# waldstein94/Stratified-Transformer

Measured on AMD Instinct MI355X. Metric: points/sec through StratifiedAttention fwd+bwd, 100k-pt scene, higher is better.
Workload: dtype f32

## Files before the change

stratified_transformer_amd/csrc/cell_attn.hip:

```cpp
#include "cell_common.h"

namespace p2 {


template <typename T>
__device__ __forceinline__ void stage_table_t(T *lds, const T *__restrict__ tab, int L, int h, int head) {
    const int total = 3 * L * 16;
    for (int x = threadIdx.x; x < total; x += blockDim.x) {
        const int i = x % 16, r = (x / 16) % L, ax = x / (16 * L);
        lds[x] = tab[(((size_t)r * h + head) * 16 + i) * 3 + ax];
    }
}
template <int TS, typename T>
__device__ __forceinline__ void stage_tables(T *lds, const T *__restrict__ table_q, const T *__restrict__ table_k, const T *__restrict__ table_v, int L,
                                             int h, int head) {
    stage_table_t<T>(lds, table_q, L, h, head);
    stage_table_t<T>(lds + TS, table_k, L, h, head);
    stage_table_t<T>(lds + 2 * TS, table_v, L, h, head);
    __syncthreads();
}

template <int LCAP>
struct TabGeo {
    static constexpr int TS = 3 * LCAP * 16;
    static constexpr size_t bytes(size_t elem) { return (size_t)3 * TS * elem; }
};
struct RowOff {
    int o0, o1, o2;
};
__device__ __forceinline__ RowOff row_off(unsigned w, int L, int c) {
    RowOff r;
    r.o0 = (int)(w & 255u) * 16 + 4 * c;
    r.o1 = (int)(L + ((w >> 8) & 255u)) * 16 + 4 * c;
    r.o2 = (int)(2 * L + ((w >> 16) & 255u)) * 16 + 4 * c;
    return r;
}
template <int OFF>
__device__ __forceinline__ float4 tsum_at(const float *lds, RowOff r) {
    return add4(add4(*reinterpret_cast<const float4 *>(lds + OFF + r.o0), *reinterpret_cast<const float4 *>(lds + OFF + r.o1)),
                *reinterpret_cast<const float4 *>(lds + OFF + r.o2));
}

struct Rows3 {
    float4 a, b, c;
};
template <int OFF, typename T>
__device__ __forceinline__ Rows3 rows_at(const T *lds, RowOff r) {
    Rows3 x;
    x.a = ld_row4(lds + OFF + r.o0);
    x.b = ld_row4(lds + OFF + r.o1);
    x.c = ld_row4(lds + OFF + r.o2);
    return x;
}
typedef float f32x2c __attribute__((ext_vector_type(2)));
__device__ __forceinline__ float4 padd4(float4 a, float4 b) {
    const f32x2c lo = f32x2c{a.x, a.y} + f32x2c{b.x, b.y}, hi = f32x2c{a.z, a.w} + f32x2c{b.z, b.w};
    return make_float4(lo.x, lo.y, hi.x, hi.y);
}
__device__ __forceinline__ float4 pfma4(float s, float4 a, float4 acc) {
    const f32x2c ss = f32x2c{s, s};
    const f32x2c lo = __builtin_elementwise_fma(ss, f32x2c{a.x, a.y}, f32x2c{acc.x, acc.y});
    const f32x2c hi = __builtin_elementwise_fma(ss, f32x2c{a.z, a.w}, f32x2c{acc.z, acc.w});
    return make_float4(lo.x, lo.y, hi.x, hi.y);
}
__device__ __forceinline__ float4 rsum(Rows3 r) { return padd4(padd4(r.a, r.b), r.c); }
__device__ __forceinline__ f32x2c pdot_acc(float4 a, float4 b, f32x2c acc) {
    acc = __builtin_elementwise_fma(f32x2c{a.x, a.y}, f32x2c{b.x, b.y}, acc);
    return __builtin_elementwise_fma(f32x2c{a.z, a.w}, f32x2c{b.z, b.w}, acc);
}
__device__ __forceinline__ float pdot4(float4 a, float4 b) {
    const f32x2c r = pdot_acc(a, b, f32x2c{0.f, 0.f});
    return r.x + r.y;
}

template <int NPMAX, typename F>
__device__ __forceinline__ void dispatch_passes(int np, F f) {
    if (np <= 2) f(std::integral_constant<int, 2>{});
    else if (np == 3) f(std::integral_constant<int, 3>{});
    else if (np == 4 || NPMAX <= 4) f(std::integral_constant<int, 4>{});
    else if constexpr (NPMAX > 4) {
        if (np <= 6) f(std::integral_constant<int, 6>{});
        else f(std::integral_constant<int, 8>{});
    }
}

template <typename TT, bool PK>
struct LaneCtx {
    const TT *lds;
    int L, lane, p, c, head, h, C, hoff, rs_packed;
    float qscale;
    __device__ __forceinline__ int rs() const { return PK ? rs_packed : C; }
    template <typename RT>
    __device__ __forceinline__ float4 q_row4(const RT *q, int i) const {
        if constexpr (PK) return scaled_row4<RT>(q + (size_t)i * rs_packed + hoff, qscale);
        else return ld_row4(q + (size_t)i * C + hoff);
    }
};
template <typename TT, bool PK>
__device__ __forceinline__ LaneCtx<TT, PK> make_lane_ctx(const TT *lds, int h, int L, int rs, float qscale) {
    LaneCtx<TT, PK> x;
    x.lds = lds;
    x.L = L;
    x.h = h;
    x.head = blockIdx.y;
    x.C = h * 16;
    x.rs_packed = rs;
    x.qscale = qscale;
    x.lane = threadIdx.x & 63;
    x.p = x.lane >> 2;
    x.c = x.lane & 3;
    x.hoff = x.head * 16 + 4 * x.c;
    return x;
}

template <int NPA, typename RT, typename T, bool PK>
__device__ __forceinline__ void load_key_rows(const LaneCtx<T, PK> &x, const CellBufs &cb, const RT *__restrict__ rows, int j0, int nvalid,
                                              float4 (&r4)[NPA]) {
    unsigned keys[NPA];
    bload_words<NPA>(cb.key, (j0 + x.p * NPA) * 4, keys);
#pragma unroll
    for (int t = 0; t < NPA; t++) {
        const float4 r = ld_row4(rows + (size_t)keys[t] * x.rs() + x.hoff);
        r4[t] = t < nvalid ? r : make_float4(0.f, 0.f, 0.f, 0.f);
    }
}

template <int NPA, int TS, typename RT, typename T, bool PK>
__device__ __forceinline__ void fwd_sweep_logits(const LaneCtx<T, PK> &x, const CellTask &ct, const CellBufs &cb, rsrc_t rs_p,
                                                 const RT *__restrict__ q, const RT *__restrict__ k, float *__restrict__ ml,
                                                 int ch, bool single, int j0, int nkc) {
    const int p = x.p, c = x.c;
    const int nvalid = min(max(nkc - p * NPA, 0), NPA);
    float4 k4[NPA];
    load_key_rows<NPA, RT, T, PK>(x, cb, k, j0, nvalid, k4);
    int ids = (int)bload_u32(cb.qid, x.lane * 4);
    int i_nx = __builtin_amdgcn_readlane(ids, 0);
    float4 q4_nx = x.q_row4(q, i_nx);
    unsigned w_nx[NPA];
    bload_words<NPA>(cb.rel, (j0 + p * NPA) * 4, w_nx);
    for (int il = 0; il < ct.nq; il++) {
        const int i = i_nx;
        const float4 q4 = q4_nx;
        unsigned w[NPA];
#pragma unroll
        for (int t = 0; t < NPA; t++) w[t] = w_nx[t];
        const int roff = (il * ct.nk + j0 + p * NPA) * 4;
        if (((il + 1) & 63) == 0) ids = (int)bload_u32(cb.qid, (il + 1 + x.lane) * 4);
        i_nx = __builtin_amdgcn_readlane(ids, (il + 1) & 63);
        q4_nx = x.q_row4(q, i_nx);
        bload_words<NPA>(cb.rel, roff + ct.nk * 4, w_nx);
        float lg[NPA];
        float mx = -INFINITY;
        RowOff ro = row_off(w[0], x.L, c);
        Rows3 rq = rows_at<0, T>(x.lds, ro), rk = rows_at<TS, T>(x.lds, ro);
#pragma unroll
        for (int t = 0; t < NPA; t++) {
            Rows3 rq1 = rq, rk1 = rk;
            if (t + 1 < NPA) {
                ro = row_off(w[t + 1], x.L, c);
                rq1 = rows_at<0, T>(x.lds, ro);
                rk1 = rows_at<TS, T>(x.lds, ro);
            }
            const f32x2c d2 = pdot_acc(k4[t], rsum(rk), pdot_acc(q4, rsum(rq), pdot_acc(q4, k4[t], f32x2c{0.f, 0.f})));
            const float s = quad_sum(d2.x + d2.y);
            lg[t] = (t < nvalid && !(w[t] >> 31)) ? s : -INFINITY;
            mx = fmaxf(mx, lg[t]);
            rq = rq1;
            rk = rk1;
            __builtin_amdgcn_sched_barrier(0);
        }
        mx = slots_max16(mx);
        if (single) {
            float sum = 0.f;
#pragma unroll
            for (int t = 0; t < NPA; t++) {
                lg[t] = __expf(lg[t] - mx);
                sum += lg[t];
            }
            const float inv = 1.0f / slots_sum16(sum);
#pragma unroll
            for (int t = 0; t < NPA; t++) lg[t] *= inv;
            if (c == 0) bstore_floats<NPA>(rs_p, roff, lg, nvalid);
        } else {
            float *st = ml + ((size_t)i * x.h + x.head) * 2;
            const float m_old = ch ? st[0] : -INFINITY, l_old = ch ? st[1] : 0.f;
            const float m_new = fmaxf(m_old, mx);
            float sum = 0.f;
#pragma unroll
            for (int t = 0; t < NPA; t++) sum += __expf(lg[t] - m_new);
            if (c == 0) bstore_floats<NPA>(rs_p, roff, lg, nvalid);
            sum = slots_sum16(sum);
            if (x.lane == 0) {
                st[0] = m_new;
                st[1] = (m_old == -INFINITY ? 0.f : l_old * __expf(m_old - m_new)) + sum;
            }
        }
    }
}

template <int NPA, int TS, typename RT, typename T, bool PK>
__device__ __forceinline__ void fwd_sweep_values(const LaneCtx<T, PK> &x, const CellTask &ct, const CellBufs &cb, rsrc_t rs_p,
                                                 const RT *__restrict__ v, const float *__restrict__ ml, float *__restrict__ out,
                                                 int ch, bool single, int j0, int nkc) {
    const int p = x.p, c = x.c;
    const int nvalid = min(max(nkc - p * NPA, 0), NPA);
    float4 v4[NPA];
    load_key_rows<NPA, RT, T, PK>(x, cb, v, j0, nvalid, v4);
    unsigned w_nx[NPA];
    float a_nx[NPA];
    bload_words<NPA>(cb.rel, (j0 + p * NPA) * 4, w_nx);
    bload_floats<NPA>(rs_p, (j0 + p * NPA) * 4, a_nx);
    int ids = (int)bload_u32(cb.qid, x.lane * 4);
    for (int il = 0; il < ct.nq; il++) {
        if (il && (il & 63) == 0) ids = (int)bload_u32(cb.qid, (il + x.lane) * 4);
        const int i = __builtin_amdgcn_readlane(ids, il & 63);
        const int roff = (il * ct.nk + j0 + p * NPA) * 4;
        unsigned w[NPA];
        float a[NPA];
#pragma unroll
        for (int t = 0; t < NPA; t++) {
            w[t] = w_nx[t];
            a[t] = a_nx[t];
        }
        bload_words<NPA>(cb.rel, roff + ct.nk * 4, w_nx);
        bload_floats<NPA>(rs_p, roff + ct.nk * 4, a_nx);
        if (!single) {
            const float *st = ml + ((size_t)i * x.h + x.head) * 2;
            const float m = st[0], inv = 1.0f / st[1];
#pragma unroll
            for (int t = 0; t < NPA; t++) a[t] = __expf(a[t] - m) * inv;
            if (c == 0) bstore_floats<NPA>(rs_p, roff, a, nvalid);
        }
        float4 acc = make_float4(0.f, 0.f, 0.f, 0.f);
        Rows3 rv = rows_at<2 * TS, T>(x.lds, row_off(w[0], x.L, c));
#pragma unroll
        for (int t = 0; t < NPA; t++) {
            Rows3 rv1 = rv;
            if (t + 1 < NPA) rv1 = rows_at<2 * TS, T>(x.lds, row_off(w[t + 1], x.L, c));
            const float at = t < nvalid ? a[t] : 0.f;
            acc = pfma4(at, padd4(rsum(rv), v4[t]), acc);
            rv = rv1;
            __builtin_amdgcn_sched_barrier(0);
        }
        const float4 tot = slots_sum16_4(acc);
        if (p == 0) {
            float *o = out + (size_t)i * x.C + x.hoff;
            stg4(o, ch ? add4(tot, ldg4(o)) : tot);
        }
    }
}

template <int NP, int LCAP, typename RT, typename T, bool PK>
__global__ __launch_bounds__(CA_WAVES * 64) void cell_fwd_kernel(pointops2_cell_plan pl, int h, int L, const RT *__restrict__ q,
                                                                 const RT *__restrict__ k, const RT *__restrict__ v, int rs, float qscale,
                                                                 const T *__restrict__ table_q, const T *__restrict__ table_k,
                                                                 const T *__restrict__ table_v, float *__restrict__ out,
                                                                 float *__restrict__ ml, float *__restrict__ pbuf, size_t plane) {
    constexpr int TS = TabGeo<LCAP>::TS;
    extern __shared__ float lds_raw[];
    T *lds = reinterpret_cast<T *>(lds_raw);
    const LaneCtx<T, PK> x = make_lane_ctx<T, PK>(lds, h, L, rs, qscale);
    const int wave = __builtin_amdgcn_readfirstlane(threadIdx.x >> 6);
    stage_tables<TS, T>(lds, table_q, table_k, table_v, L, h, x.head);
    const int nC = share_count(pl, pl.counts[0]);
    float *pb = pbuf + (size_t)x.head * plane;
    const int slots = gridDim.x * CA_WAVES, slot = blockIdx.x * CA_WAVES + wave;
    for (int round = 0; round * slots < nC; round++) {
        const int task = snake_task(round, slot, slots);
        if (task >= nC) continue;
        const CellTask ct = cell_task(pl, share_task(pl, task));
        const int nch = (ct.nk + 16 * NP - 1) / (16 * NP);
        const CellBufs cb = make_cell_bufs(pl, ct);
        const rsrc_t rs_p = tile_rsrc(pb, ct);
        for (int ch = 0; ch < nch; ch++) {
            const int j0 = ch * 16 * NP, nkc = min(16 * NP, ct.nk - j0);
            dispatch_passes<NP>((nkc + 15) >> 4, [&](auto tag) {
                fwd_sweep_logits<decltype(tag)::value, TS, RT, T, PK>(x, ct, cb, rs_p, q, k, ml, ch, nch == 1, j0, nkc);
            });
        }
        for (int ch = 0; ch < nch; ch++) {
            const int j0 = ch * 16 * NP, nkc = min(16 * NP, ct.nk - j0);
            dispatch_passes<NP>((nkc + 15) >> 4, [&](auto tag) {
                fwd_sweep_values<decltype(tag)::value, TS, RT, T, PK>(x, ct, cb, rs_p, v, ml, out, ch, nch == 1, j0, nkc);
            });
        }
    }
}

template <int NPA, typename T, bool PK>
__device__ __forceinline__ void flush_key_pass(float *scr, float4 acc, rsrc_t rs_key, int j0, int t, int nkc, float *__restrict__ grad,
                                               const LaneCtx<T, PK> &x) {
    *reinterpret_cast<float4 *>(scr + x.p * 16 + 4 * x.c) = acc;
    __builtin_amdgcn_s_waitcnt(0xC07F);
    __builtin_amdgcn_wave_barrier();
#pragma unroll
    for (int kk = 0; kk < 4; kk++) {
        const int s = (x.lane >> 4) + 4 * kk;
        const int jl = s * NPA + t;
        const int key = (int)bload_u32(rs_key, (j0 + jl) * 4);
        if (jl < nkc) unsafeAtomicAdd(grad + (size_t)key * x.rs() + x.head * 16 + (x.lane & 15), scr[s * 16 + (x.lane & 15)]);
    }
    __builtin_amdgcn_s_waitcnt(0xC07F);
    __builtin_amdgcn_wave_barrier();
}

template <int NPA, int TS, typename RT, typename T, bool PK>
__device__ __forceinline__ void bwd_sweep_values(const LaneCtx<T, PK> &x, const CellTask &ct, const CellBufs &cb, rsrc_t rs_p, rsrc_t rs_g,
                                                 float *scr, const float *__restrict__ go, const float *__restrict__ out,
                                                 const RT *__restrict__ v, float *__restrict__ grad_v, int j0, int nkc) {
    const int p = x.p, c = x.c;
    const int nvalid = min(max(nkc - p * NPA, 0), NPA);
    float4 v4[NPA], dv4[NPA];
    load_key_rows<NPA, RT, T, PK>(x, cb, v, j0, nvalid, v4);
#pragma unroll
    for (int t = 0; t < NPA; t++) dv4[t] = make_float4(0.f, 0.f, 0.f, 0.f);
    unsigned w_nx[NPA];
    float a_nx[NPA];
    bload_words<NPA>(cb.rel, (j0 + p * NPA) * 4, w_nx);
    bload_floats<NPA>(rs_p, (j0 + p * NPA) * 4, a_nx);
    int ids = (int)bload_u32(cb.qid, x.lane * 4);
    int i_nx = __builtin_amdgcn_readlane(ids, 0);
    float4 go_nx = ldg4(go + (size_t)i_nx * x.C + x.hoff), o_nx = ldg4(out + (size_t)i_nx * x.C + x.hoff);
    for (int il = 0; il < ct.nq; il++) {
        const int roff = (il * ct.nk + j0 + p * NPA) * 4;
        const float4 go4 = go_nx, o4 = o_nx;
        unsigned w[NPA];
        float a[NPA];
#pragma unroll
        for (int t = 0; t < NPA; t++) {
            w[t] = w_nx[t];
            a[t] = t < nvalid ? a_nx[t] : 0.f;
        }
        if (((il + 1) & 63) == 0) ids = (int)bload_u32(cb.qid, (il + 1 + x.lane) * 4);
        i_nx = __builtin_amdgcn_readlane(ids, (il + 1) & 63);
        go_nx = ldg4(go + (size_t)i_nx * x.C + x.hoff);
        o_nx = ldg4(out + (size_t)i_nx * x.C + x.hoff);
        bload_words<NPA>(cb.rel, roff + ct.nk * 4, w_nx);
        bload_floats<NPA>(rs_p, roff + ct.nk * 4, a_nx);
        const float delta = quad_sum(pdot4(go4, o4));
        float gs[NPA];
        Rows3 rv = rows_at<2 * TS, T>(x.lds, row_off(w[0], x.L, c));
#pragma unroll
        for (int t = 0; t < NPA; t++) {
            Rows3 rv1 = rv;
            if (t + 1 < NPA) rv1 = rows_at<2 * TS, T>(x.lds, row_off(w[t + 1], x.L, c));
            const float ga = quad_sum(pdot4(go4, padd4(rsum(rv), v4[t])));
            gs[t] = a[t] * (ga - delta);
            dv4[t] = pfma4(a[t], go4, dv4[t]);
            rv = rv1;
            __builtin_amdgcn_sched_barrier(0);
        }
        if (c == 0) bstore_floats<NPA>(rs_g, roff, gs, nvalid);
    }
#pragma unroll
    for (int t = 0; t < NPA; t++) flush_key_pass<NPA, T, PK>(scr, dv4[t], cb.key, j0, t, nkc, grad_v, x);
}

template <int NPA, int TS, typename RT, typename T, bool PK>
__device__ __forceinline__ void bwd_sweep_keys(const LaneCtx<T, PK> &x, const CellTask &ct, const CellBufs &cb, rsrc_t rs_g, float *scr,
                                               const RT *__restrict__ q, const RT *__restrict__ k, float *__restrict__ grad_q,
                                               float *__restrict__ grad_k, int ch, int j0, int nkc) {
    const int p = x.p, c = x.c;
    const int nvalid = min(max(nkc - p * NPA, 0), NPA);
    float4 k4[NPA], dk4[NPA];
    load_key_rows<NPA, RT, T, PK>(x, cb, k, j0, nvalid, k4);
#pragma unroll
    for (int t = 0; t < NPA; t++) dk4[t] = make_float4(0.f, 0.f, 0.f, 0.f);
    unsigned w_nx[NPA];
    float g_nx[NPA];
    bload_words<NPA>(cb.rel, (j0 + p * NPA) * 4, w_nx);
    bload_floats<NPA>(rs_g, (j0 + p * NPA) * 4, g_nx);
    int ids = (int)bload_u32(cb.qid, x.lane * 4);
    int i_nx = __builtin_amdgcn_readlane(ids, 0);
    float4 q_nx = x.q_row4(q, i_nx);
    for (int il = 0; il < ct.nq; il++) {
        const int i = i_nx;
        const int roff = (il * ct.nk + j0 + p * NPA) * 4;
        const float4 q4 = q_nx;
        unsigned w[NPA];
        float g[NPA];
#pragma unroll
        for (int t = 0; t < NPA; t++) {
            w[t] = w_nx[t];
            g[t] = t < nvalid ? g_nx[t] : 0.f;
        }
        if (((il + 1) & 63) == 0) ids = (int)bload_u32(cb.qid, (il + 1 + x.lane) * 4);
        i_nx = __builtin_amdgcn_readlane(ids, (il + 1) & 63);
        q_nx = x.q_row4(q, i_nx);
        bload_words<NPA>(cb.rel, roff + ct.nk * 4, w_nx);
        bload_floats<NPA>(rs_g, roff + ct.nk * 4, g_nx);
        float4 dq = make_float4(0.f, 0.f, 0.f, 0.f);
        RowOff ro = row_off(w[0], x.L, c);
        Rows3 rq = rows_at<0, T>(x.lds, ro), rk = rows_at<TS, T>(x.lds, ro);
#pragma unroll
        for (int t = 0; t < NPA; t++) {
            Rows3 rq1 = rq, rk1 = rk;
            if (t + 1 < NPA) {
                ro = row_off(w[t + 1], x.L, c);
                rq1 = rows_at<0, T>(x.lds, ro);
                rk1 = rows_at<TS, T>(x.lds, ro);
            }
            dq = pfma4(g[t], padd4(rsum(rq), k4[t]), dq);
            dk4[t] = pfma4(g[t], padd4(rsum(rk), q4), dk4[t]);
            rq = rq1;
            rk = rk1;
            __builtin_amdgcn_sched_barrier(0);
        }
        float4 tot = slots_sum16_4(dq);
        if constexpr (PK) tot = make_float4(tot.x * x.qscale, tot.y * x.qscale, tot.z * x.qscale, tot.w * x.qscale);
        if (p == 0) {
            float *o = grad_q + (size_t)i * x.rs() + x.hoff;
            stg4(o, ch ? add4(tot, ldg4(o)) : tot);
        }
    }
#pragma unroll
    for (int t = 0; t < NPA; t++) flush_key_pass<NPA, T, PK>(scr, dk4[t], cb.key, j0, t, nkc, grad_k, x);
}

template <int NP, int LCAP, typename RT, typename T, bool PK>
__global__ __launch_bounds__(CA_WAVES_BWD * 64) void cell_bwd_kernel(pointops2_cell_plan pl, int h, int L, const float *__restrict__ go,
                                                                 const RT *__restrict__ q, const RT *__restrict__ k,
                                                                 const RT *__restrict__ v, int rs, float qscale, const float *__restrict__ out,
                                                                 const T *__restrict__ table_q, const T *__restrict__ table_k,
                                                                 const T *__restrict__ table_v, const float *__restrict__ pbuf,
                                                                 float *__restrict__ gsbuf, size_t plane, float *__restrict__ grad_q,
                                                                 float *__restrict__ grad_k, float *__restrict__ grad_v) {
    constexpr int TS = TabGeo<LCAP>::TS;
    extern __shared__ float lds_raw[];
    T *lds = reinterpret_cast<T *>(lds_raw);
    const LaneCtx<T, PK> x = make_lane_ctx<T, PK>(lds, h, L, rs, qscale);
    const int wave = __builtin_amdgcn_readfirstlane(threadIdx.x >> 6);
    float *scr = reinterpret_cast<float *>(lds + 3 * TS) + wave * 256;
    stage_tables<TS, T>(lds, table_q, table_k, table_v, L, h, x.head);
    const int nC = share_count(pl, pl.counts[0]);
    const float *pb = pbuf + (size_t)x.head * plane;
    float *gb = gsbuf + (size_t)x.head * plane;
    const int slots = gridDim.x * CA_WAVES_BWD, slot = blockIdx.x * CA_WAVES_BWD + wave;
    for (int round = 0; round * slots < nC; round++) {
        const int task = snake_task(round, slot, slots);
        if (task >= nC) continue;
        const CellTask ct = cell_task(pl, share_task(pl, task));
        const int nch = (ct.nk + 16 * NP - 1) / (16 * NP);
        const CellBufs cb = make_cell_bufs(pl, ct);
        const rsrc_t rs_p = tile_rsrc(pb, ct), rs_g = tile_rsrc(gb, ct);
        for (int ch = 0; ch < nch; ch++) {
            const int j0 = ch * 16 * NP, nkc = min(16 * NP, ct.nk - j0);
            dispatch_passes<NP>((nkc + 15) >> 4, [&](auto tag) {
                bwd_sweep_values<decltype(tag)::value, TS, RT, T, PK>(x, ct, cb, rs_p, rs_g, scr, go, out, v, grad_v, j0, nkc);
            });
        }
        for (int ch = 0; ch < nch; ch++) {
            const int j0 = ch * 16 * NP, nkc = min(16 * NP, ct.nk - j0);
            dispatch_passes<NP>((nkc + 15) >> 4, [&](auto tag) {
                bwd_sweep_keys<decltype(tag)::value, TS, RT, T, PK>(x, ct, cb, rs_g, scr, q, k, grad_q, grad_k, ch, j0, nkc);
            });
        }
    }
}

struct CFixScale {
    float mul, inv;
};
__device__ __forceinline__ CFixScale c_row_scale(unsigned maxbits, int n) {
    CFixScale sc;
    if (maxbits >= 0x7f800000u) {
        sc.mul = 0.f;
        sc.inv = __uint_as_float(0x7fc00000u);
        return sc;
    }
    const int E = (int)(maxbits >> 23) - 126;
    const int bits_n = 32 - __clz(max(n, 1));
    const int S = max(-126, min(126, 30 - bits_n - E));
    sc.mul = __uint_as_float((unsigned)(S + 127) << 23);
    sc.inv = __uint_as_float((unsigned)(127 - S) << 23);
    return sc;
}

constexpr int CT_WAVES = 8;

template <int TA>
struct CellTableGeo {
    static constexpr int LP = TA * 16;
    static constexpr int ROW = 3 * LP + 16;
    static constexpr size_t walk_bytes() { return (size_t)CT_WAVES * 4 * ROW * 4; }
    static constexpr size_t sum_bytes() { return (size_t)LP * 48 * 4; }
    static constexpr size_t lds_bytes() { return walk_bytes() > sum_bytes() ? walk_bytes() : sum_bytes(); }
};

template <int TA, bool BYKEY, bool SC, typename XT>
__device__ __forceinline__ void cell_table_grad_body(const pointops2_cell_plan &pl, int h, int L, const float *__restrict__ wbuf, size_t plane,
                                                     const XT *__restrict__ X, int xs, float xscale, float *__restrict__ grad_table) {
    constexpr int D = 16;
    constexpr int MAXP = BYKEY ? 4 : 8;
    using G = CellTableGeo<TA>;
    extern __shared__ float lds[];
    const int wave = __builtin_amdgcn_readfirstlane(threadIdx.x >> 6), lane = threadIdx.x & 63;
    const int head = blockIdx.y;
    const int p = lane >> 2, c = lane & 3;
    const int kq = lane >> 4, col = lane & 15;
    int *hist = reinterpret_cast<int *>(lds) + wave * 4 * G::ROW;
    const float *wb = wbuf + (size_t)head * plane;

    f32x4c acc[TA][3];
#pragma unroll
    for (int bt = 0; bt < TA; bt++)
#pragma unroll
        for (int ax = 0; ax < 3; ax++) acc[bt][ax] = f32x4c{0.f, 0.f, 0.f, 0.f};
    for (int x = lane; x < 4 * G::ROW; x += 64) hist[x] = 0;

    const int nC = BYKEY ? pl.counts[4] : share_count(pl, pl.counts[0]);
    const int slots = gridDim.x * CT_WAVES, slot = blockIdx.x * CT_WAVES + wave;
    for (int round = 0; round * slots < nC; round++) {
        const int task = snake_task(round, slot, slots);
        if (task >= nC) continue;
        CellTask ct;
        if (BYKEY) {
            const int c0 = __builtin_amdgcn_readfirstlane(pl.parent_first[task]), c1 = __builtin_amdgcn_readfirstlane(pl.parent_first[task + 1]);
            ct.qs = __builtin_amdgcn_readfirstlane(pl.cell_qstart[c0]);
            ct.nq = __builtin_amdgcn_readfirstlane(pl.cell_qstart[c1]) - ct.qs;
            ct.kb = __builtin_amdgcn_readfirstlane(pl.cell_kbase[c0]);
            ct.nk = __builtin_amdgcn_readfirstlane(pl.cell_kbase[c0 + 1]) - ct.kb;
            ct.pbase = __builtin_amdgcn_readfirstlane(pl.cell_pbase[c0]);
        } else {
            ct = cell_task(pl, share_task(pl, task));
        }
        const CellBufs cb = make_cell_bufs(pl, ct);
        const rsrc_t rs_rel = cb.rel, rs_w = tile_rsrc(wb, ct), rs_row = BYKEY ? cb.key : cb.qid;
        const int nrows = BYKEY ? ct.nk : ct.nq, nent = BYKEY ? ct.nq : ct.nk;
        auto entry_off = [&](int r0, int ent) -> int { return (BYKEY ? ent * ct.nk + r0 + c : (r0 + c) * ct.nk + ent) * 4; };
        auto consume = [&](int r0, int e0, float xv, unsigned (&wr)[MAXP], float (&wt)[MAXP]) {
            const int ne = min(nent - e0, 16 * MAXP);
            const bool row_ok = r0 + c < nrows;
            unsigned mxb = 0u;
#pragma unroll
            for (int t = 0; t < MAXP; t++) {
                const bool live = row_ok && e0 + 16 * t + p < nent && !(wr[t] >> 31);
                wt[t] = live ? wt[t] : 0.f;
                mxb = max(mxb, __float_as_uint(fabsf(wt[t])));
            }
            const CFixScale sc = c_row_scale(wave_max_u32(mxb), ne);
            int *myh = hist + c * G::ROW;
#pragma unroll
            for (int t = 0; t < MAXP; t++) {
                if (16 * t < ne && wt[t] != 0.f) {
                    const int v = __float2int_rn(wt[t] * sc.mul);
                    atomicAdd(&myh[wr[t] & 255u], v);
                    atomicAdd(&myh[G::LP + ((wr[t] >> 8) & 255u)], v);
                    atomicAdd(&myh[2 * G::LP + ((wr[t] >> 16) & 255u)], v);
                }
            }
            __builtin_amdgcn_s_waitcnt(0xC07F);
            __builtin_amdgcn_wave_barrier();
            const float b = xv * sc.inv;
#pragma unroll
            for (int bt = 0; bt < TA; bt++)
#pragma unroll
                for (int ax = 0; ax < 3; ax++) {
                    const float a = (float)__hip_atomic_exchange(&hist[kq * G::ROW + ax * G::LP + bt * 16 + col], 0, __ATOMIC_RELAXED,
                                                                 __HIP_MEMORY_SCOPE_WORKGROUP);
                    acc[bt][ax] = __builtin_amdgcn_mfma_f32_16x16x4f32(a, b, acc[bt][ax], 0, 0, 0);
                }
            __builtin_amdgcn_s_waitcnt(0xC07F);
            __builtin_amdgcn_wave_barrier();
        };
        unsigned wr_n[MAXP];
        float wt_n[MAXP];
#pragma unroll
        for (int t = 0; t < MAXP; t++) {
            wr_n[t] = 0x80000000u;
            wt_n[t] = 0.f;
            if (16 * t < nent) {
                wr_n[t] = bload_u32(rs_rel, entry_off(0, 16 * t + p));
                wt_n[t] = bload_f32(rs_w, entry_off(0, 16 * t + p));
            }
        }
        int pt_n = (int)bload_u32(rs_row, kq * 4);
        float xv_n = SC ? scaled_elem<XT>(X + (size_t)pt_n * xs + head * D + col, xscale) : ld_elem(X + (size_t)pt_n * xs + head * D + col);
        pt_n = (int)bload_u32(rs_row, (4 + kq) * 4);
        for (int r0 = 0; r0 < nrows; r0 += 4) {
            unsigned wr[MAXP];
            float wt[MAXP];
#pragma unroll
            for (int t = 0; t < MAXP; t++) {
                wr[t] = wr_n[t];
                wt[t] = wt_n[t];
            }
            const float xv = r0 + kq < nrows ? xv_n : 0.f;
            xv_n = SC ? scaled_elem<XT>(X + (size_t)pt_n * xs + head * D + col, xscale) : ld_elem(X + (size_t)pt_n * xs + head * D + col);
            pt_n = (int)bload_u32(rs_row, (r0 + 8 + kq) * 4);
#pragma unroll
            for (int t = 0; t < MAXP; t++)
                if (16 * t < nent) {
                    wr_n[t] = bload_u32(rs_rel, entry_off(r0 + 4, 16 * t + p));
                    wt_n[t] = bload_f32(rs_w, entry_off(r0 + 4, 16 * t + p));
                }
            consume(r0, 0, xv, wr, wt);
            for (int e0 = 16 * MAXP; e0 < nent; e0 += 16 * MAXP) {
#pragma unroll
                for (int t = 0; t < MAXP; t++) {
                    wr[t] = bload_u32(rs_rel, entry_off(r0, e0 + 16 * t + p));
                    wt[t] = bload_f32(rs_w, entry_off(r0, e0 + 16 * t + p));
                }
                consume(r0, e0, xv, wr, wt);
            }
        }
    }
    __syncthreads();
    float *sum = lds;
    for (int w = 0; w < CT_WAVES; w++) {
        if (wave == w) {
#pragma unroll
            for (int bt = 0; bt < TA; bt++)
#pragma unroll
                for (int ax = 0; ax < 3; ax++)
#pragma unroll
                    for (int reg = 0; reg < 4; reg++) {
                        float *d = &sum[((bt * 16 + kq * 4 + reg) * 16 + col) * 3 + ax];
                        *d = w ? *d + acc[bt][ax][reg] : acc[bt][ax][reg];
                    }
        }
        __syncthreads();
    }
    for (int x = threadIdx.x; x < L * 48; x += CT_WAVES * 64) {
        const float val = sum[x];
        if (val != 0.f) unsafeAtomicAdd(grad_table + ((size_t)(x / 48) * h + head) * 48 + x % 48, val);
    }
}

template <int TA, typename T, bool PK>
__global__ __launch_bounds__(CT_WAVES * 64) void cell_table_grad3_kernel(pointops2_cell_plan pl, int h, int L, const float *__restrict__ gsbuf,
                                                                         const float *__restrict__ pbuf, size_t plane,
                                                                         const T *__restrict__ q, const T *__restrict__ k,
                                                                         const float *__restrict__ grad_out, float *__restrict__ gtq,
                                                                         float *__restrict__ gtk, float *__restrict__ gtv, int rs, float qscale) {
    const int xs = PK ? rs : h * 16;
    if (blockIdx.z == 0) cell_table_grad_body<TA, true, false, T>(pl, h, L, gsbuf, plane, k, xs, 1.0f, gtk);
    else if (blockIdx.z == 1) cell_table_grad_body<TA, false, PK, T>(pl, h, L, gsbuf, plane, q, xs, qscale, gtq);
    else cell_table_grad_body<TA, false, false, float>(pl, h, L, pbuf, plane, grad_out, h * 16, 1.0f, gtv);
}

static const char *cell_refusal(const pointops2_cell_plan *plan, int hdim, int L, bool backward) {
    if (hdim != 16) return "cell_attention: d != 16";
    if (backward && (L < 1 || L > 80)) return "cell_attention backward: table rows L must be in 1..80";
    if (L < 1) return "cell_attention: no table rows";
    if (L != plan->table_rows)
        return backward ? "cell_attention backward: the tables' row count differs from the plan's table_rows"
                        : "cell_attention: the tables' row count differs from the plan's table_rows";
    if (L > 160) return "cell_attention: more than 160 table rows (use the operators)";
    return nullptr;
}

static int cell_fwd_variant(const pointops2_cell_plan *plan, int h, int hdim, int L, bool bf16, const char **why) {
    *why = nullptr;
    if (plan == nullptr || plan->n_points <= 0) return POINTOPS2_CELL_FWD_NONE;
    if ((*why = cell_refusal(plan, hdim, L, false)) != nullptr) return POINTOPS2_CELL_FWD_ERROR;
    if (L > 80) return POINTOPS2_CELL_FWD_VALU160;
    if (!bf16) {
        const double avg_queries = (double)plan->n_pairs / (double)(plan->n_keyslots > 0 ? plan->n_keyslots : 1);
        if (!((long long)plan->n_points * h >= 96000 && avg_queries < 15.0)) return L <= 64 ? POINTOPS2_CELL_FWD_MFMA64 : POINTOPS2_CELL_FWD_MFMA80;
    }
    return POINTOPS2_CELL_FWD_VALU80;
}

template <int LCAP, typename RT, typename TT, bool PK>
static void launch_valu_fwd(hipStream_t st, const pointops2_cell_plan *plan, int h, int L, const CellRows<RT> &r, const CellTables<TT> &t, float *out, float *ml,
                            float *pbuf) {
    const size_t lds = TabGeo<LCAP>::bytes(sizeof(TT));
    allow_big_lds(cell_fwd_kernel<CA_NP, LCAP, RT, TT, PK>, lds);
    const dim3 grid(cell_grid_x(1, plan->n_cells, h, CA_WAVES), h);
    hipLaunchKernelGGL((cell_fwd_kernel<CA_NP, LCAP, RT, TT, PK>), grid, dim3(CA_WAVES * 64), lds, st, *plan, h, L, r.q, r.k, r.v, r.rs, r.scale, t.q, t.k, t.v, out,
                       ml, pbuf, (size_t)plan->n_pairs);
}

template <typename RT, typename TT, bool PK>
static void launch_cell_fwd(hipStream_t st, const pointops2_cell_plan *plan, int h, int hdim, int L, const CellRows<RT> &r, const CellTables<TT> &t, float *out,
                            float *ml, float *pbuf) {
    const char *why;
    const int variant = cell_fwd_variant(plan, h, hdim, L, !std::is_same<TT, float>::value, &why);
    if (why != nullptr) { set_error(why); return; }
    if (variant == POINTOPS2_CELL_FWD_NONE) return;
    if constexpr (std::is_same<TT, float>::value) {
        if (variant == POINTOPS2_CELL_FWD_MFMA64 || variant == POINTOPS2_CELL_FWD_MFMA80) {
            cell_fwd_mfma_launch(st, variant, plan, h, L, RowTag<RT>::code, PK, CellRows<void>{r.q, r.k, r.v, r.rs, r.scale}, t, out, pbuf);
            check_launch();
            return;
        }
    }
    if (variant == POINTOPS2_CELL_FWD_VALU80) launch_valu_fwd<80, RT, TT, PK>(st, plan, h, L, r, t, out, ml, pbuf);
    else launch_valu_fwd<160, RT, TT, PK>(st, plan, h, L, r, t, out, ml, pbuf);
    check_launch();
}

template <typename RT, typename TT, bool PK>
static void launch_cell_bwd(hipStream_t st, const pointops2_cell_plan *plan, int h, int hdim, int L, const float *grad_out, const CellRows<RT> &r, const float *out,
                            const CellTables<TT> &t, const float *pbuf, float *gsbuf, const CellGrads &g, const CellGrads &gt) {
    if (plan == nullptr || plan->n_points <= 0) return;
    if (const char *why = cell_refusal(plan, hdim, L, true)) { set_error(why); return; }
    const size_t lds = TabGeo<80>::bytes(sizeof(TT)) + (size_t)CA_WAVES_BWD * 256 * sizeof(float);
    allow_big_lds(cell_bwd_kernel<CA_NP_BWD, 80, RT, TT, PK>, lds);
    const size_t plane = (size_t)plan->n_pairs;
    hipLaunchKernelGGL((cell_bwd_kernel<CA_NP_BWD, 80, RT, TT, PK>), dim3(cell_grid_x(1, plan->n_cells, h, CA_WAVES_BWD), h),
                       dim3(CA_WAVES_BWD * 64), lds, st, *plan, h, L, grad_out, r.q, r.k, r.v, r.rs, r.scale, out, t.q, t.k, t.v, pbuf, gsbuf, plane, g.q, g.k, g.v);
    const dim3 grid3(cell_grid_x(1, plan->n_cells, h, CT_WAVES), h, 3), tblock(CT_WAVES * 64);
    if (L <= 64) hipLaunchKernelGGL((cell_table_grad3_kernel<4, RT, PK>), grid3, tblock, CellTableGeo<4>::lds_bytes(), st, *plan, h, L, gsbuf, pbuf, plane, r.q, r.k,
                                    grad_out, gt.q, gt.k, gt.v, r.rs, r.scale);
    else hipLaunchKernelGGL((cell_table_grad3_kernel<5, RT, PK>), grid3, tblock, CellTableGeo<5>::lds_bytes(), st, *plan, h, L, gsbuf, pbuf, plane, r.q, r.k, grad_out,
                            gt.q, gt.k, gt.v, r.rs, r.scale);
    check_launch();
}

template <typename RT>
static CellRows<RT> packed_rows(const void *qkv, int h, float scale) {
    const RT *r = static_cast<const RT *>(qkv);
    return {r, r + h * 16, r + 2 * h * 16, 3 * h * 16, scale};
}

}

using namespace p2;

extern "C" {

int pointops2_cell_forward_variant(const pointops2_cell_plan *plan, int h, int hdim, int L, int bf16) {
    const char *why;
    return cell_fwd_variant(plan, h, hdim, L, bf16 != 0, &why);
}

void cell_attention_forward_launcher(const pointops2_cell_plan *plan, int h, int hdim, int L, const float *q, const float *k,
                                     const float *v, const float *table_q, const float *table_k, const float *table_v, float *out,
                                     float *ml, float *pbuf) {
    launch_cell_fwd<float, float, false>(begin_launch().stream, plan, h, hdim, L, {q, k, v, h * 16, 1.0f}, {table_q, table_k, table_v}, out, ml, pbuf);
}
void cell_attention_backward_launcher(const pointops2_cell_plan *plan, int h, int hdim, int L, const float *grad_out, const float *q,
                                      const float *k, const float *v, const float *out, const float *table_q, const float *table_k,
                                      const float *table_v, const float *pbuf, float *gsbuf, float *grad_q, float *grad_k,
                                      float *grad_v, float *grad_table_q, float *grad_table_k, float *grad_table_v) {
    launch_cell_bwd<float, float, false>(begin_launch().stream, plan, h, hdim, L, grad_out, {q, k, v, h * 16, 1.0f}, out, {table_q, table_k, table_v}, pbuf, gsbuf,
                                         {grad_q, grad_k, grad_v}, {grad_table_q, grad_table_k, grad_table_v});
}
void cell_attention_forward_bf16_launcher(const pointops2_cell_plan *plan, int h, int hdim, int L, const uint16_t *q, const uint16_t *k,
                                          const uint16_t *v, const uint16_t *table_q, const uint16_t *table_k, const uint16_t *table_v,
                                          float *out, float *ml, float *pbuf) {
    launch_cell_fwd<bf16_t, bf16_t, false>(begin_launch().stream, plan, h, hdim, L, {q, k, v, h * 16, 1.0f}, {table_q, table_k, table_v}, out, ml, pbuf);
}
void cell_attention_backward_bf16_launcher(const pointops2_cell_plan *plan, int h, int hdim, int L, const float *grad_out, const uint16_t *q,
                                           const uint16_t *k, const uint16_t *v, const float *out, const uint16_t *table_q,
                                           const uint16_t *table_k, const uint16_t *table_v, const float *pbuf, float *gsbuf, float *grad_q,
                                           float *grad_k, float *grad_v, float *grad_table_q, float *grad_table_k, float *grad_table_v) {
    launch_cell_bwd<bf16_t, bf16_t, false>(begin_launch().stream, plan, h, hdim, L, grad_out, {q, k, v, h * 16, 1.0f}, out, {table_q, table_k, table_v}, pbuf, gsbuf,
                                           {grad_q, grad_k, grad_v}, {grad_table_q, grad_table_k, grad_table_v});
}

void cell_attention_qkv_forward_launcher(const pointops2_cell_plan *plan, int h, int hdim, int L, const void *qkv, int row_type, float scale,
                                         const float *table_q, const float *table_k, const float *table_v, float *out, float *ml, float *pbuf) {
    const hipStream_t st = begin_launch().stream;
    if (!with_row_type(row_type, [&](auto tag) {
        using RT = typename decltype(tag)::type;
        launch_cell_fwd<RT, float, true>(st, plan, h, hdim, L, packed_rows<RT>(qkv, h, scale), {table_q, table_k, table_v}, out, ml, pbuf);
    })) set_error("cell_attention_qkv: unknown row_type");
}
void cell_attention_qkv_backward_launcher(const pointops2_cell_plan *plan, int h, int hdim, int L, const float *grad_out, const void *qkv, int row_type,
                                          float scale, const float *out, const float *table_q, const float *table_k, const float *table_v,
                                          const float *pbuf, float *gsbuf, float *grad_qkv, float *grad_table_q, float *grad_table_k,
                                          float *grad_table_v) {
    const hipStream_t st = begin_launch().stream;
    if (!with_row_type(row_type, [&](auto tag) {
        using RT = typename decltype(tag)::type;
        launch_cell_bwd<RT, float, true>(st, plan, h, hdim, L, grad_out, packed_rows<RT>(qkv, h, scale), out, {table_q, table_k, table_v}, pbuf, gsbuf,
                                         {grad_qkv, grad_qkv + h * 16, grad_qkv + 2 * h * 16}, {grad_table_q, grad_table_k, grad_table_v});
    })) set_error("cell_attention_qkv backward: unknown row_type");
}

}
```

Measured before the change: 8.750 million.

## Process eight key columns per wave in key-table gradient walk

Splits the by-key path of the table-gradient kernel into its own function. Each wave now handles KC=8 key columns per pass instead of 4, with a per-column histogram and a shuffle-based max reduction over partial wave groups. The aim is more reuse per load and less loop overhead in the key-table gradient. In exchange it doubles the per-wave histogram LDS, which raises the kernel's shared-memory footprint and may cut occupancy for every z-slice.

```diff
diff --git a/stratified_transformer_amd/csrc/cell_attn.hip b/stratified_transformer_amd/csrc/cell_attn.hip
--- a/stratified_transformer_amd/csrc/cell_attn.hip
+++ b/stratified_transformer_amd/csrc/cell_attn.hip
@@ -478,20 +478,47 @@
 
 constexpr int CT_WAVES = 8;
 
+constexpr int CT_KCOLS = 8;
+
 template <int TA>
 struct CellTableGeo {
     static constexpr int LP = TA * 16;
     static constexpr int ROW = 3 * LP + 16;
-    static constexpr size_t walk_bytes() { return (size_t)CT_WAVES * 4 * ROW * 4; }
+    static constexpr size_t walk_bytes(int rows) { return (size_t)CT_WAVES * rows * ROW * 4; }
     static constexpr size_t sum_bytes() { return (size_t)LP * 48 * 4; }
-    static constexpr size_t lds_bytes() { return walk_bytes() > sum_bytes() ? walk_bytes() : sum_bytes(); }
+    static constexpr size_t lds_bytes(int rows) { return walk_bytes(rows) > sum_bytes() ? walk_bytes(rows) : sum_bytes(); }
 };
 
-template <int TA, bool BYKEY, bool SC, typename XT>
+template <int TA>
+__device__ __forceinline__ void table_grad_flush(const f32x4c (&acc)[TA][3], float *sum, int wave, int L, int h, int head,
+                                                 float *__restrict__ grad_table) {
+    const int kq = (threadIdx.x & 63) >> 4, col = threadIdx.x & 15;
+    __syncthreads();
+    for (int w = 0; w < CT_WAVES; w++) {
+        if (wave == w) {
+#pragma unroll
+            for (int bt = 0; bt < TA; bt++)
+#pragma unroll
+                for (int ax = 0; ax < 3; ax++)
+#pragma unroll
+                    for (int reg = 0; reg < 4; reg++) {
+                        float *d = &sum[((bt * 16 + kq * 4 + reg) * 16 + col) * 3 + ax];
+                        *d = w ? *d + acc[bt][ax][reg] : acc[bt][ax][reg];
+                    }
+        }
+        __syncthreads();
+    }
+    for (int x = threadIdx.x; x < L * 48; x += CT_WAVES * 64) {
+        const float val = sum[x];
+        if (val != 0.f) unsafeAtomicAdd(grad_table + ((size_t)(x / 48) * h + head) * 48 + x % 48, val);
+    }
+}
+
+template <int TA, bool SC, typename XT>
 __device__ __forceinline__ void cell_table_grad_body(const pointops2_cell_plan &pl, int h, int L, const float *__restrict__ wbuf, size_t plane,
                                                      const XT *__restrict__ X, int xs, float xscale, float *__restrict__ grad_table) {
     constexpr int D = 16;
-    constexpr int MAXP = BYKEY ? 4 : 8;
+    constexpr int MAXP = 8;
     using G = CellTableGeo<TA>;
     extern __shared__ float lds[];
     const int wave = __builtin_amdgcn_readfirstlane(threadIdx.x >> 6), lane = threadIdx.x & 63;
@@ -508,26 +535,16 @@
         for (int ax = 0; ax < 3; ax++) acc[bt][ax] = f32x4c{0.f, 0.f, 0.f, 0.f};
     for (int x = lane; x < 4 * G::ROW; x += 64) hist[x] = 0;
 
-    const int nC = BYKEY ? pl.counts[4] : share_count(pl, pl.counts[0]);
+    const int nC = share_count(pl, pl.counts[0]);
     const int slots = gridDim.x * CT_WAVES, slot = blockIdx.x * CT_WAVES + wave;
     for (int round = 0; round * slots < nC; round++) {
         const int task = snake_task(round, slot, slots);
         if (task >= nC) continue;
-        CellTask ct;
-        if (BYKEY) {
-            const int c0 = __builtin_amdgcn_readfirstlane(pl.parent_first[task]), c1 = __builtin_amdgcn_readfirstlane(pl.parent_first[task + 1]);
-            ct.qs = __builtin_amdgcn_readfirstlane(pl.cell_qstart[c0]);
-            ct.nq = __builtin_amdgcn_readfirstlane(pl.cell_qstart[c1]) - ct.qs;
-            ct.kb = __builtin_amdgcn_readfirstlane(pl.cell_kbase[c0]);
-            ct.nk = __builtin_amdgcn_readfirstlane(pl.cell_kbase[c0 + 1]) - ct.kb;
-            ct.pbase = __builtin_amdgcn_readfirstlane(pl.cell_pbase[c0]);
-        } else {
-            ct = cell_task(pl, share_task(pl, task));
-        }
+        const CellTask ct = cell_task(pl, share_task(pl, task));
         const CellBufs cb = make_cell_bufs(pl, ct);
-        const rsrc_t rs_rel = cb.rel, rs_w = tile_rsrc(wb, ct), rs_row = BYKEY ? cb.key : cb.qid;
-        const int nrows = BYKEY ? ct.nk : ct.nq, nent = BYKEY ? ct.nq : ct.nk;
-        auto entry_off = [&](int r0, int ent) -> int { return (BYKEY ? ent * ct.nk + r0 + c : (r0 + c) * ct.nk + ent) * 4; };
+        const rsrc_t rs_rel = cb.rel, rs_w = tile_rsrc(wb, ct), rs_row = cb.qid;
+        const int nrows = ct.nq, nent = ct.nk;
+        auto entry_off = [&](int r0, int ent) -> int { return ((r0 + c) * ct.nk + ent) * 4; };
         auto consume = [&](int r0, int e0, float xv, unsigned (&wr)[MAXP], float (&wt)[MAXP]) {
             const int ne = min(nent - e0, 16 * MAXP);
             const bool row_ok = r0 + c < nrows;
@@ -605,26 +622,143 @@
             }
         }
     }
-    __syncthreads();
-    float *sum = lds;
-    for (int w = 0; w < CT_WAVES; w++) {
-        if (wave == w) {
-#pragma unroll
-            for (int bt = 0; bt < TA; bt++)
-#pragma unroll
-                for (int ax = 0; ax < 3; ax++)
-#pragma unroll
-                    for (int reg = 0; reg < 4; reg++) {
-                        float *d = &sum[((bt * 16 + kq * 4 + reg) * 16 + col) * 3 + ax];
-                        *d = w ? *d + acc[bt][ax][reg] : acc[bt][ax][reg];
+    table_grad_flush<TA>(acc, lds, wave, L, h, head, grad_table);
+}
+
+template <int TA, int KC, typename XT>
+__device__ __forceinline__ void cell_table_grad_keys(const pointops2_cell_plan &pl, int h, int L, const float *__restrict__ wbuf, size_t plane,
+                                                     const XT *__restrict__ X, int xs, float *__restrict__ grad_table) {
+    static_assert(KC == 4 || KC == 8 || KC == 16, "whole groups of four columns, whole query rows per load");
+    constexpr int D = 16;
+    constexpr int NG = KC / 4;
+    constexpr int QP = 64 / KC;
+    constexpr int MAXP = KC == 16 ? 8 : 4;
+    using G = CellTableGeo<TA>;
+    extern __shared__ float lds[];
+    const int wave = __builtin_amdgcn_readfirstlane(threadIdx.x >> 6), lane = threadIdx.x & 63;
+    const int head = blockIdx.y;
+    const int p = lane / KC, c = lane % KC;
+    const int kq = lane >> 4, col = lane & 15;
+    int *hist = reinterpret_cast<int *>(lds) + wave * KC * G::ROW;
+    const float *wb = wbuf + (size_t)head * plane;
+
+    f32x4c acc[TA][3];
+#pragma unroll
+    for (int bt = 0; bt < TA; bt++)
+#pragma unroll
+        for (int ax = 0; ax < 3; ax++) acc[bt][ax] = f32x4c{0.f, 0.f, 0.f, 0.f};
+    for (int x = lane; x < KC * G::ROW; x += 64) hist[x] = 0;
+
+    const int nC = pl.counts[4];
+    const int slots = gridDim.x * CT_WAVES, slot = blockIdx.x * CT_WAVES + wave;
+    for (int round = 0; round * slots < nC; round++) {
+        const int task = snake_task(round, slot, slots);
+        if (task >= nC) continue;
+        CellTask ct;
+        const int c0 = __builtin_amdgcn_readfirstlane(pl.parent_first[task]), c1 = __builtin_amdgcn_readfirstlane(pl.parent_first[task + 1]);
+        ct.qs = __builtin_amdgcn_readfirstlane(pl.cell_qstart[c0]);
+        ct.nq = __builtin_amdgcn_readfirstlane(pl.cell_qstart[c1]) - ct.qs;
+        ct.kb = __builtin_amdgcn_readfirstlane(pl.cell_kbase[c0]);
+        ct.nk = __builtin_amdgcn_readfirstlane(pl.cell_kbase[c0 + 1]) - ct.kb;
+        ct.pbase = __builtin_amdgcn_readfirstlane(pl.cell_pbase[c0]);
+        const CellBufs cb = make_cell_bufs(pl, ct);
+        const rsrc_t rs_rel = cb.rel, rs_w = tile_rsrc(wb, ct), rs_key = cb.key;
+        const int nk = ct.nk, nq = ct.nq;
+        auto entry_off = [&](int r0, int e) -> int { return (e * nk + r0 + c) * 4; };
+        auto consume = [&](int r0, int e0, const float (&xv)[NG], unsigned (&wr)[MAXP], float (&wt)[MAXP]) {
+            const int ne = min(nq - e0, QP * MAXP);
+            const bool col_ok = r0 + c < nk;
+            unsigned mxb = 0u;
+#pragma unroll
+            for (int t = 0; t < MAXP; t++) {
+                const bool live = col_ok && e0 + QP * t + p < nq && !(wr[t] >> 31);
+                wt[t] = live ? wt[t] : 0.f;
+                mxb = max(mxb, __float_as_uint(fabsf(wt[t])));
+            }
+#pragma unroll
+            for (int m = KC; m < 64; m <<= 1) mxb = max(mxb, (unsigned)__shfl_xor((int)mxb, m, 64));
+            const CFixScale sc = c_row_scale(mxb, ne);
+            int *myh = hist + c * G::ROW;
+#pragma unroll
+            for (int t = 0; t < MAXP; t++) {
+                if (QP * t < ne && wt[t] != 0.f) {
+                    const int v = __float2int_rn(wt[t] * sc.mul);
+                    atomicAdd(&myh[wr[t] & 255u], v);
+                    atomicAdd(&myh[G::LP + ((wr[t] >> 8) & 255u)], v);
+                    atomicAdd(&myh[2 * G::LP + ((wr[t] >> 16) & 255u)], v);
+                }
+            }
+            __builtin_amdgcn_s_waitcnt(0xC07F);
+            __builtin_amdgcn_wave_barrier();
+#pragma unroll
+            for (int g = 0; g < NG; g++) {
+                if (r0 + 4 * g >= nk) break;
+                const float b = xv[g] * __shfl(sc.inv, 4 * g + kq, 64);
+                const int *hg = hist + (4 * g + kq) * G::ROW + col;
+#pragma unroll
+                for (int bt = 0; bt < TA; bt++)
+#pragma unroll
+                    for (int ax = 0; ax < 3; ax++) {
+                        const float a = (float)__hip_atomic_exchange(const_cast<int *>(&hg[ax * G::LP + bt * 16]), 0, __ATOMIC_RELAXED,
+                                                                     __HIP_MEMORY_SCOPE_WORKGROUP);
+                        acc[bt][ax] = __builtin_amdgcn_mfma_f32_16x16x4f32(a, b, acc[bt][ax], 0, 0, 0);
                     }
-        }
-        __syncthreads();
-    }
-    for (int x = threadIdx.x; x < L * 48; x += CT_WAVES * 64) {
-        const float val = sum[x];
-        if (val != 0.f) unsafeAtomicAdd(grad_table + ((size_t)(x / 48) * h + head) * 48 + x % 48, val);
-    }
+            }
+            __builtin_amdgcn_s_waitcnt(0xC07F);
+            __builtin_amdgcn_wave_barrier();
+        };
+        unsigned wr_n[MAXP];
+        float wt_n[MAXP];
+#pragma unroll
+        for (int t = 0; t < MAXP; t++) {
+            wr_n[t] = 0x80000000u;
+            wt_n[t] = 0.f;
+            if (QP * t < nq) {
+                wr_n[t] = bload_u32(rs_rel, entry_off(0, QP * t + p));
+                wt_n[t] = bload_f32(rs_w, entry_off(0, QP * t + p));
+            }
+        }
+        int pt_n[NG];
+        float xv_n[NG];
+#pragma unroll
+        for (int g = 0; g < NG; g++) pt_n[g] = (int)bload_u32(rs_key, (4 * g + kq) * 4);
+#pragma unroll
+        for (int g = 0; g < NG; g++) {
+            xv_n[g] = ld_elem(X + (size_t)pt_n[g] * xs + head * D + col);
+            pt_n[g] = (int)bload_u32(rs_key, (KC + 4 * g + kq) * 4);
+        }
+        for (int r0 = 0; r0 < nk; r0 += KC) {
+            unsigned wr[MAXP];
+            float wt[MAXP], xv[NG];
+#pragma unroll
+            for (int t = 0; t < MAXP; t++) {
+                wr[t] = wr_n[t];
+                wt[t] = wt_n[t];
+            }
+#pragma unroll
+            for (int g = 0; g < NG; g++) {
+                xv[g] = r0 + 4 * g + kq < nk ? xv_n[g] : 0.f;
+                xv_n[g] = ld_elem(X + (size_t)pt_n[g] * xs + head * D + col);
+                pt_n[g] = (int)bload_u32(rs_key, (r0 + 2 * KC + 4 * g + kq) * 4);
+            }
+#pragma unroll
+            for (int t = 0; t < MAXP; t++)
+                if (QP * t < nq) {
+                    wr_n[t] = bload_u32(rs_rel, entry_off(r0 + KC, QP * t + p));
+                    wt_n[t] = bload_f32(rs_w, entry_off(r0 + KC, QP * t + p));
+                }
+            consume(r0, 0, xv, wr, wt);
+            for (int e0 = QP * MAXP; e0 < nq; e0 += QP * MAXP) {
+#pragma unroll
+                for (int t = 0; t < MAXP; t++) {
+                    wr[t] = bload_u32(rs_rel, entry_off(r0, e0 + QP * t + p));
+                    wt[t] = bload_f32(rs_w, entry_off(r0, e0 + QP * t + p));
+                }
+                consume(r0, e0, xv, wr, wt);
+            }
+        }
+    }
+    table_grad_flush<TA>(acc, lds, wave, L, h, head, grad_table);
 }
 
 template <int TA, typename T, bool PK>
@@ -634,9 +768,9 @@
                                                                          const float *__restrict__ grad_out, float *__restrict__ gtq,
                                                                          float *__restrict__ gtk, float *__restrict__ gtv, int rs, float qscale) {
     const int xs = PK ? rs : h * 16;
-    if (blockIdx.z == 0) cell_table_grad_body<TA, true, false, T>(pl, h, L, gsbuf, plane, k, xs, 1.0f, gtk);
-    else if (blockIdx.z == 1) cell_table_grad_body<TA, false, PK, T>(pl, h, L, gsbuf, plane, q, xs, qscale, gtq);
-    else cell_table_grad_body<TA, false, false, float>(pl, h, L, pbuf, plane, grad_out, h * 16, 1.0f, gtv);
+    if (blockIdx.z == 0) cell_table_grad_keys<TA, CT_KCOLS, T>(pl, h, L, gsbuf, plane, k, xs, gtk);
+    else if (blockIdx.z == 1) cell_table_grad_body<TA, PK, T>(pl, h, L, gsbuf, plane, q, xs, qscale, gtq);
+    else cell_table_grad_body<TA, false, float>(pl, h, L, pbuf, plane, grad_out, h * 16, 1.0f, gtv);
 }
 
 static const char *cell_refusal(const pointops2_cell_plan *plan, int hdim, int L, bool backward) {
@@ -691,6 +825,15 @@
     check_launch();
 }
 
+template <int TA, typename RT, bool PK>
+static void launch_table_grad3(hipStream_t st, dim3 grid, dim3 block, const pointops2_cell_plan *plan, int h, int L, const float *grad_out, const CellRows<RT> &r,
+                               const float *pbuf, const float *gsbuf, size_t plane, const CellGrads &gt) {
+    constexpr size_t lds = CellTableGeo<TA>::lds_bytes(CT_KCOLS);
+    allow_big_lds(cell_table_grad3_kernel<TA, RT, PK>, lds);
+    hipLaunchKernelGGL((cell_table_grad3_kernel<TA, RT, PK>), grid, block, lds, st, *plan, h, L, gsbuf, pbuf, plane, r.q, r.k, grad_out, gt.q, gt.k, gt.v, r.rs,
+                       r.scale);
+}
+
 template <typename RT, typename TT, bool PK>
 static void launch_cell_bwd(hipStream_t st, const pointops2_cell_plan *plan, int h, int hdim, int L, const float *grad_out, const CellRows<RT> &r, const float *out,
                             const CellTables<TT> &t, const float *pbuf, float *gsbuf, const CellGrads &g, const CellGrads &gt) {
@@ -702,10 +845,8 @@
     hipLaunchKernelGGL((cell_bwd_kernel<CA_NP_BWD, 80, RT, TT, PK>), dim3(cell_grid_x(1, plan->n_cells, h, CA_WAVES_BWD), h),
                        dim3(CA_WAVES_BWD * 64), lds, st, *plan, h, L, grad_out, r.q, r.k, r.v, r.rs, r.scale, out, t.q, t.k, t.v, pbuf, gsbuf, plane, g.q, g.k, g.v);
     const dim3 grid3(cell_grid_x(1, plan->n_cells, h, CT_WAVES), h, 3), tblock(CT_WAVES * 64);
-    if (L <= 64) hipLaunchKernelGGL((cell_table_grad3_kernel<4, RT, PK>), grid3, tblock, CellTableGeo<4>::lds_bytes(), st, *plan, h, L, gsbuf, pbuf, plane, r.q, r.k,
-                                    grad_out, gt.q, gt.k, gt.v, r.rs, r.scale);
-    else hipLaunchKernelGGL((cell_table_grad3_kernel<5, RT, PK>), grid3, tblock, CellTableGeo<5>::lds_bytes(), st, *plan, h, L, gsbuf, pbuf, plane, r.q, r.k, grad_out,
-                            gt.q, gt.k, gt.v, r.rs, r.scale);
+    if (L <= 64) launch_table_grad3<4, RT, PK>(st, grid3, tblock, plan, h, L, grad_out, r, pbuf, gsbuf, plane, gt);
+    else launch_table_grad3<5, RT, PK>(st, grid3, tblock, plan, h, L, grad_out, r, pbuf, gsbuf, plane, gt);
     check_launch();
 }
 
```

Result: slower. 7.351 million (-16.0%).
